# scorbiclife/LifeAPI

Measured on AMD Instinct MI355X. Metric: 64x64 universe-generations/sec (+ cell-updates/sec) at 1/2/4/8 MI355X, higher is better.
Workload: dtype u64

## Files before the change

### lifeapi_amd/csrc/device.hpp

```cpp
#pragma once

#include <hip/hip_runtime.h>

#include <cstdint>

#include "common.hpp"

namespace lifeapi_impl {


struct W {
  uint32_t lo, hi;
};

__device__ __forceinline__ W split(uint64_t v) { return W{(uint32_t)v, (uint32_t)(v >> 32)}; }
__device__ __forceinline__ uint64_t join(W w) { return (uint64_t)w.lo | ((uint64_t)w.hi << 32); }

__device__ __forceinline__ W rot_up(W a) {
  return W{__builtin_amdgcn_alignbit(a.lo, a.hi, 31), __builtin_amdgcn_alignbit(a.hi, a.lo, 31)};
}
__device__ __forceinline__ W rot_dn(W a) {
  return W{__builtin_amdgcn_alignbit(a.hi, a.lo, 1), __builtin_amdgcn_alignbit(a.lo, a.hi, 1)};
}

constexpr uint32_t TA = 0xF0, TB = 0xCC, TC = 0xAA;
constexpr uint32_t kXor3 = (TA ^ TB ^ TC) & 0xFF;
constexpr uint32_t kMaj = ((TA & TB) | (TA & TC) | (TB & TC)) & 0xFF;
constexpr uint32_t kCarry2 = (TA ^ (TB & TC)) & 0xFF;
constexpr uint32_t kLive = ((TA ^ TB) & (TC | TA)) & 0xFF;

template <uint32_t TT>
__device__ __forceinline__ uint32_t lut3(uint32_t a, uint32_t b, uint32_t c) {
  return __builtin_amdgcn_bitop3_b32(a, b, c, TT);
}
template <uint32_t TT>
__device__ __forceinline__ W lut3(W a, W b, W c) {
  return W{lut3<TT>(a.lo, b.lo, c.lo), lut3<TT>(a.hi, b.hi, c.hi)};
}


enum Xchg { XDPP = 0, XLDS = 1, XBPERM = 2, XMIX = 3, XMIX1 = 4, XMIX3 = 5, XLDSR = 6, XLDSR3 = 7, XASM = 8 };
constexpr bool uses_lds(int x) { return x == XLDS || x == XLDSR || x == XLDSR3 || x == XASM; }

__device__ __forceinline__ uint32_t dpp_prev(uint32_t v) {
  return (uint32_t)__builtin_amdgcn_mov_dpp((int)v, 0x13C, 0xF, 0xF, true);
}
__device__ __forceinline__ uint32_t dpp_next(uint32_t v) {
  return (uint32_t)__builtin_amdgcn_mov_dpp((int)v, 0x134, 0xF, 0xF, true);
}
__device__ __forceinline__ uint32_t bperm_prev(uint32_t v, int lane) {
  return (uint32_t)__builtin_amdgcn_ds_bpermute(((lane + kWave - 1) & (kWave - 1)) << 2, (int)v);
}
__device__ __forceinline__ uint32_t bperm_next(uint32_t v, int lane) {
  return (uint32_t)__builtin_amdgcn_ds_bpermute(((lane + 1) & (kWave - 1)) << 2, (int)v);
}

template <int X>
__device__ __forceinline__ void neighbour_cols(W a, W &L, W &R, uint64_t *slot, int lane);

template <int X>
__device__ __forceinline__ void neighbours(W c0, W c1, W &L0, W &R0, W &L1, W &R1,
                                           uint64_t *slot, int lane) {
  if constexpr (X != XLDS) {
    neighbour_cols<X>(c0, L0, R0, slot, lane);
    neighbour_cols<X>(c1, L1, R1, slot, lane);
  } else {
    uint64_t *s = slot;
    s[lane] = join(c0);
    s[kWave + lane] = join(c1);
    __builtin_amdgcn_wave_barrier();
    const int xp = (lane + kWave - 1) & (kWave - 1), xn = (lane + 1) & (kWave - 1);
    L0 = split(s[xp]);
    R0 = split(s[xn]);
    L1 = split(s[kWave + xp]);
    R1 = split(s[kWave + xn]);
    __builtin_amdgcn_wave_barrier();
  }
}

template <int X>
__device__ __forceinline__ void neighbour_cols(W a, W &L, W &R, uint64_t *slot, int lane) {
  if constexpr (X == XDPP) {
    L = W{dpp_prev(a.lo), dpp_prev(a.hi)};
    R = W{dpp_next(a.lo), dpp_next(a.hi)};
  } else if constexpr (X == XBPERM) {
    L = W{bperm_prev(a.lo, lane), bperm_prev(a.hi, lane)};
    R = W{bperm_next(a.lo, lane), bperm_next(a.hi, lane)};
  } else if constexpr (X == XMIX) {
    L = W{dpp_prev(a.lo), dpp_prev(a.hi)};
    R = W{bperm_next(a.lo, lane), bperm_next(a.hi, lane)};
  } else if constexpr (X == XMIX1) {
    L = W{dpp_prev(a.lo), dpp_prev(a.hi)};
    R = W{dpp_next(a.lo), bperm_next(a.hi, lane)};
  } else if constexpr (X == XMIX3) {
    L = W{dpp_prev(a.lo), bperm_prev(a.hi, lane)};
    R = W{bperm_next(a.lo, lane), bperm_next(a.hi, lane)};
  } else if constexpr (X == XLDSR || X == XLDSR3) {
    uint64_t *s = slot;
    s[lane] = join(a);
    __builtin_amdgcn_wave_barrier();
    R = split(s[(lane + 1) & (kWave - 1)]);
    if constexpr (X == XLDSR) {
      L = W{dpp_prev(a.lo), dpp_prev(a.hi)};
    } else {
      const uint32_t *s32 = reinterpret_cast<const uint32_t *>(s);
      L = W{dpp_prev(a.lo), s32[2 * ((lane + kWave - 1) & (kWave - 1)) + 1]};
    }
    __builtin_amdgcn_wave_barrier();
  } else {
    uint64_t *s = slot;
    s[lane] = join(a);
    __builtin_amdgcn_wave_barrier();
    L = split(s[(lane + kWave - 1) & (kWave - 1)]);
    R = split(s[(lane + 1) & (kWave - 1)]);
    __builtin_amdgcn_wave_barrier();
  }
}

constexpr uint32_t kLe1 = (~kMaj) & 0xFF;
constexpr uint32_t kNae = ((TA ^ TB) | (TB ^ TC)) & 0xFF;
constexpr uint32_t kEven = (~kXor3) & 0xFF;
constexpr uint32_t kT1 = 0x34, kT2 = 0x58, kT3 = 0x28;

constexpr uint32_t kN1 = 0xE9, kN4 = 0x52, kN6 = 0xE0;
__device__ __forceinline__ uint32_t life_tail6(uint32_t h0u, uint32_t h0, uint32_t h0d, uint32_t h1u,
                                               uint32_t h1, uint32_t h1d, uint32_t a) {
  const uint32_t g1 = lut3<kN1>(h1, h1u, h1d);
  const uint32_t g2 = lut3<kMaj>(h1d, h1u, h0d);
  const uint32_t g3 = lut3<kNae>(h0d, h0u, h0);
  const uint32_t g4 = lut3<kN4>(g3, g2, g1);
  const uint32_t g5 = lut3<kXor3>(h0, h0d, h0u);
  return lut3<kN6>(g4, g5, a);
}
__device__ __forceinline__ uint32_t life_tail7(uint32_t h0u, uint32_t h0, uint32_t h0d, uint32_t h1u,
                                               uint32_t h1, uint32_t h1d, uint32_t a) {
  const uint32_t s0 = lut3<kLe1>(h0u, h0, h0d), s1 = lut3<kNae>(h0u, h0, h0d);
  const uint32_t s2 = lut3<kLe1>(h1u, h1, h1d), s3 = lut3<kEven>(h1u, h1, h1d);
  const uint32_t t1 = lut3<kT1>(s0, s1, a);
  const uint32_t t2 = lut3<kT2>(s2, a, t1);
  return lut3<kT3>(s1, s3, t2);
}
template <int NET>
__device__ __forceinline__ uint32_t life_tail(uint32_t h0u, uint32_t h0, uint32_t h0d, uint32_t h1u,
                                              uint32_t h1, uint32_t h1d, uint32_t a) {
  static_assert(NET == 6 || NET == 7, "tails: 6 or 7 LUTs");
  if constexpr (NET == 6) return life_tail6(h0u, h0, h0d, h1u, h1, h1d, a);
  else return life_tail7(h0u, h0, h0d, h1u, h1, h1d, a);
}

typedef uint64_t u64x2 __attribute__((ext_vector_type(2)));

template <bool NT>
__device__ __forceinline__ W ld(const uint64_t *p) {
  if constexpr (NT) return split(__builtin_nontemporal_load(p));
  else return split(*p);
}
template <bool NT>
__device__ __forceinline__ void st(uint64_t *p, W v) {
  if constexpr (NT) __builtin_nontemporal_store(join(v), p);
  else *p = join(v);
}

__device__ __forceinline__ uint64_t mix64(uint64_t z) {
  z = (z ^ (z >> 30)) * 0xBF58476D1CE4E5B9ULL;
  z = (z ^ (z >> 27)) * 0x94D049BB133111EBULL;
  return z ^ (z >> 31);
}

template <int CTRL>
__device__ __forceinline__ uint32_t dpp_mov(uint32_t v) {
  return (uint32_t)__builtin_amdgcn_update_dpp(0, (int)v, CTRL, 0xF, 0xF, false);
}
template <int CTRL>
__device__ __forceinline__ uint64_t dpp_mov64(uint64_t v) {
  return (uint64_t)dpp_mov<CTRL>((uint32_t)v) | ((uint64_t)dpp_mov<CTRL>((uint32_t)(v >> 32)) << 32);
}
__device__ __forceinline__ uint32_t wave_sum_u32_dpp(uint32_t v) {
  v += dpp_mov<0xB1>(v);
  v += dpp_mov<0x4E>(v);
  v += dpp_mov<0x141>(v);
  v += dpp_mov<0x140>(v);
  return (uint32_t)__builtin_amdgcn_readlane(v, 0) + (uint32_t)__builtin_amdgcn_readlane(v, 16) +
         (uint32_t)__builtin_amdgcn_readlane(v, 32) + (uint32_t)__builtin_amdgcn_readlane(v, 48);
}
__device__ __forceinline__ uint32_t lane_id_fresh() {
  uint32_t l;
  asm volatile("v_mbcnt_lo_u32_b32 %0, -1, 0\n v_mbcnt_hi_u32_b32 %0, -1, %0" : "=v"(l));
  return l;
}

__device__ __forceinline__ uint32_t wave_or_u32_dpp(uint32_t v) {
  v |= dpp_mov<0xB1>(v);
  v |= dpp_mov<0x4E>(v);
  v |= dpp_mov<0x141>(v);
  v |= dpp_mov<0x140>(v);
  return (uint32_t)__builtin_amdgcn_readlane(v, 0) | (uint32_t)__builtin_amdgcn_readlane(v, 16) |
         (uint32_t)__builtin_amdgcn_readlane(v, 32) | (uint32_t)__builtin_amdgcn_readlane(v, 48);
}
__device__ __forceinline__ uint64_t wave_sum_u64_dpp(uint64_t v) {
  auto step = [&](auto mov) __attribute__((always_inline)) {
    v += (uint64_t)mov((uint32_t)v) | ((uint64_t)mov((uint32_t)(v >> 32)) << 32);
  };
  step(dpp_mov<0xB1>);
  step(dpp_mov<0x4E>);
  step(dpp_mov<0x141>);
  step(dpp_mov<0x140>);
  uint64_t t = 0;
#pragma unroll
  for (int r = 0; r < 4; ++r)
    t += (uint64_t)(uint32_t)__builtin_amdgcn_readlane((uint32_t)v, 16 * r) |
         ((uint64_t)(uint32_t)__builtin_amdgcn_readlane((uint32_t)(v >> 32), 16 * r) << 32);
  return t;
}

__device__ __forceinline__ uint32_t wave_sum_u32(uint32_t v) {
#pragma unroll
  for (int off = 32; off > 0; off >>= 1) v += __shfl_xor(v, off, kWave);
  return v;
}
__device__ __forceinline__ uint64_t wave_sum_u64(uint64_t v) {
#pragma unroll
  for (int off = 32; off > 0; off >>= 1) v += __shfl_xor(v, off, kWave);
  return v;
}

__device__ __forceinline__ uint32_t wave_excl_scan(uint32_t v, int lane) {
  uint32_t inc = v;
#pragma unroll
  for (int off = 1; off < kWave; off <<= 1) {
    const uint32_t t = __shfl_up(inc, off, kWave);
    if (lane >= off) inc += t;
  }
  return inc - v;
}
__device__ __forceinline__ uint64_t below_lane(int lane) { return (1ull << lane) - 1; }
__device__ __forceinline__ int last_set(uint64_t m) { return m ? 63 - __builtin_clzll(m) : -1; }


__device__ __forceinline__ uint64_t xcd_chunk_block() {
  const uint32_t b = blockIdx.x, nb = gridDim.x, q = nb >> 3, r = nb & 7u, x = b & 7u;
  return (uint64_t)x * q + (x < r ? x : r) + (b >> 3);
}
template <bool CHUNK>
__device__ __forceinline__ uint64_t block_index() {
  if constexpr (CHUNK) return xcd_chunk_block();
  else return blockIdx.x;
}

__device__ __forceinline__ uint64_t rotr64(uint64_t v, uint32_t k) {
  return (v >> k) | (v << ((64 - k) & 63));
}
__device__ __forceinline__ void care_window(uint64_t rm, uint32_t &y0, uint32_t &h) {
  y0 = 0;
  h = 1;
  if (rm == 0) return;
  uint64_t run[6];
  run[0] = ~rm;
#pragma unroll
  for (int k = 1; k < 6; ++k) run[k] = run[k - 1] & rotr64(run[k - 1], 1u << (k - 1));
  uint64_t cur = ~0ull;
  uint32_t len = 0;
#pragma unroll
  for (int k = 5; k >= 0; --k) {
    const uint64_t t = cur & rotr64(run[k], len);
    if (t) cur = t, len += 1u << k;
  }
  h = 64 - len;
  y0 = len ? ((uint32_t)__builtin_ctzll(cur) + len) & 63 : 0;
}
constexpr int kWaitVm0 = 0x0F70, kWaitVm1 = 0x0F71, kWaitVm5 = 0x0F75, kWaitVm6 = 0x0F76, kWaitVm9 = 0x0F79,
              kWaitVm11 = 0x0F7B, kWaitLgkm0 = 0xC07F;

__device__ __forceinline__ bool wave_contains(W s, W w, W u) {
  const uint32_t dlo = (s.lo ^ w.lo) & (w.lo | u.lo), dhi = (s.hi ^ w.hi) & (w.hi | u.hi);
  return __ballot((dlo | dhi) != 0u) == 0ull;
}


}
```

### lifeapi_amd/csrc/step.hip

```cpp
#include <algorithm>

#include "cone_launch.hpp"
#include "contains_kernels.hpp"
#include "launch.hpp"
#include "step_kernels.hpp"

using namespace lifeapi_impl;

namespace {

using StepFn = void (*)(const uint64_t *, uint64_t *, uint64_t, uint32_t, uint64_t);

constexpr uint64_t kCachedUniverses = 1ull << 22;
constexpr uint64_t kCap7Universes = 1ull << 20;
constexpr uint64_t kCap6Universes = 1ull << 21;
constexpr int kStreamResidentBlocks = 6;
int stream_resident_blocks(uint64_t n) {
  return n < kCap7Universes ? 0 : n < kCap6Universes ? 7 : kStreamResidentBlocks;
}
constexpr uint64_t kOrderMinUniverses = 3ull << 16;
constexpr uint64_t kPlainBytes = 256ull << 20;
constexpr uint64_t kFilterOrderUniverses = 1ull << 21;
constexpr const char *kStreamName =
    "k_step<dpp, 4 universes/wave, nt loads, 7-LUT network; alternating order, the last min(256 MiB, half) of "
    "each launch stored plain, the rest nt>";
constexpr const char *kStreamBigName =
    "k_step<dpp, 4 universes/wave, nt, 7-LUT network; each XCD a contiguous eighth, one order>";
struct StepLaunch {
  StepFn fn;
  uint64_t universes_per_wave;
  int resident_blocks;
  bool alternate;
  uint64_t plain_bytes;
  const char *name;
  uint32_t flags;
};
StepLaunch shipped_step(uint32_t gens, uint64_t n) {
  if (gens <= 2 && n > kCachedUniverses)
    return {k_step<XDPP, 4, true, 3, true, true>, 4, stream_resident_blocks(n), false, 0, kStreamBigName, kXcdChunk};
  if (gens <= 2)
    return {k_step<XDPP, 4, true, 3, true, true>, 4, stream_resident_blocks(n), true,
            std::min<uint64_t>(kPlainBytes, n * 512 / 2), kStreamName, 0u};
  if (gens < 32)
    return {k_step_split<8, 1, true, 6, kAsmLoop>, 4, 0, false, 0,
            "k_step_split<8-way split, 4 universes/wave, nt, 6-LUT tail, assembly loop>", 0u};
  return {k_step_split<8, 1, false, 6, kAsmLoop>, 4, 0, false, 0,
          "k_step_split<8-way split, 4 universes/wave, 6-LUT tail, assembly loop>", 0u};
}


constexpr int kFilterIterBlocksPerCU = 16;
constexpr int kSplitIterBlocksPerCU = 32;

using SplitFn = void (*)(const uint64_t *, uint64_t *, const uint64_t *, const uint64_t *, uint32_t *, uint64_t,
                         uint32_t, uint32_t);

int filter_cone(const uint64_t *d_in, const uint64_t *d_wanted, const uint64_t *d_unwanted, uint32_t *d_first_gen,
                size_t n, uint32_t generations, void *stream) {
  return launch_cone_adapt<kConeSets, true, uint32_t, true>(d_in, d_wanted, d_unwanted, d_first_gen, n, generations, 0,
                                                            (hipStream_t)stream, kConeAdaptBlocksPerCU, kWave,
                                                            kConeAdaptBlocksPerCU);
}

int filter_iterated(const uint64_t *d_in, const uint64_t *d_wanted, const uint64_t *d_unwanted,
                    uint32_t *d_first_gen, size_t n, uint32_t generations, void *stream) {
  const SplitFn fn = aligned16(d_in) ? k_step_contains_split<8, kContainsNet, kContainsAll, true, true>
                                     : k_step_contains_split<8, kContainsNet, kContainsAll, false, true>;
  return launch(fn, "k_step_contains_split launch", Grid{(n + 3) / 4, kFilterIterBlocksPerCU}, stream,
                kWritesNoBatch, d_in, nullptr, d_wanted, d_unwanted, d_first_gen, n, generations, kConeIterColumns);
}

int final_split_pair(const uint64_t *d_in, uint64_t *d_final, const uint64_t *d_wanted, const uint64_t *d_unwanted,
                     uint32_t *d_first_gen, size_t n, uint32_t generations, void *stream) {
  int cus = 0, rc = device_cus(cus);
  Written w{d_final, (uint64_t)n * 512};
  for (const SplitFn fn : {SplitFn(k_step_contains_split<8, kContainsNet, kContainsLo>),
                           SplitFn(k_step_contains_split<8, kContainsNet, kContainsHi>)}) {
    if (rc != LIFEAPI_OK) return rc;
    rc = launch(fn, "k_step_contains_split launch", Grid{(n + 3) / 4, kSplitIterBlocksPerCU, 0, cus}, stream, w, d_in,
                d_final, d_wanted, d_unwanted, d_first_gen, n, generations, 0u);
    w.recorded = true;
  }
  return rc;
}

int final_stream(const uint64_t *d_in, uint64_t *d_final, const uint64_t *d_wanted, const uint64_t *d_unwanted,
                 uint32_t *d_first_gen, size_t n, uint32_t generations, void *stream) {
  const uint64_t groups = (n + 7) / 8;
  const bool keyed = n <= kFilterOrderUniverses && n >= kOrderMinUniverses;
  const LaunchOrder o = launch_order(d_in, d_final, (uint64_t)n * 512, groups, 8 * 512, keyed,
                                     keyed ? std::min<uint64_t>(kPlainBytes, n * 512 / 2) : 0);
  return launch(k_step_contains<8>, "k_step_contains launch", Grid{groups}, stream, o.written, d_in, d_final,
                d_wanted, d_unwanted, d_first_gen, n, generations | (o.reverse ? kReverse : 0u), o.plain_from);
}

}

extern "C" {

const char *lifeapi_step_kernel_name_n(uint32_t generations, size_t n) {
  return shipped_step(generations, n).name;
}
const char *lifeapi_step_kernel_name(uint32_t generations) { return shipped_step(generations, 1).name; }

int lifeapi_step_batch_dev(const uint64_t *d_in, uint64_t *d_out, size_t n, uint32_t generations,
                           void *stream) {
  int rc = check_batch(d_in, d_out, n);
  if (rc != LIFEAPI_OK || n == 0) return rc;
  const StepLaunch l = shipped_step(generations, n);
  const uint64_t waves = (n + l.universes_per_wave - 1) / l.universes_per_wave;
  const LaunchOrder o = launch_order(d_in, d_out, (uint64_t)n * 512, waves, l.universes_per_wave * 512,
                                     l.alternate && n >= kOrderMinUniverses, l.plain_bytes);
  return launch(l.fn, "k_step launch", Grid{waves, 0, l.resident_blocks, 0, true}, stream, o.written, d_in, d_out, n,
                generations | (o.reverse ? kReverse : 0u) | l.flags, o.plain_from);
}

int lifeapi_step_contains_batch_dev(const uint64_t *d_in, uint64_t *d_final,
                                    const uint64_t *d_wanted, const uint64_t *d_unwanted,
                                    uint32_t *d_first_gen, size_t n, uint32_t generations,
                                    void *stream) {
  if (n == 0) return LIFEAPI_OK;
  if (!d_in || !d_wanted || !d_unwanted || !d_first_gen || !aligned8(d_in) ||
      !aligned8(d_wanted) || !aligned8(d_unwanted) || ((uintptr_t)d_first_gen & 3u))
    return fail(LIFEAPI_E_INVALID, "bad pointer to lifeapi_step_contains_batch_dev%s");
  if (!d_final) {
    if (generations <= 2) return filter_cone(d_in, d_wanted, d_unwanted, d_first_gen, n, generations, stream);
    return filter_iterated(d_in, d_wanted, d_unwanted, d_first_gen, n, generations, stream);
  }
  const int rc = check_batch(d_in, d_final, n);
  if (rc != LIFEAPI_OK) return rc;
  if (generations > 2)
    return final_split_pair(d_in, d_final, d_wanted, d_unwanted, d_first_gen, n, generations, stream);
  return final_stream(d_in, d_final, d_wanted, d_unwanted, d_first_gen, n, generations, stream);
}

}
```

### lifeapi_amd/csrc/step_kernels.hpp

```cpp
#pragma once

#include "life_gen.hpp"
#include "split_layout.hpp"
#include "split_asm.inc"

namespace lifeapi_impl {
namespace {

constexpr uint32_t kReverse = 1u << 31;
constexpr uint32_t kXcdChunk = 1u << 30;

template <int X, int U, bool NT, int RULE, bool NTS, bool FULL>
__device__ __forceinline__ void step_group(const uint64_t *in, uint64_t *out, uint64_t n, uint32_t gens,
                                           uint64_t u0, bool nts, uint64_t *slot, int lane) {
  W a[U];
#pragma unroll
  for (int k = 0; k < U; ++k)
    a[k] = (FULL || u0 + k < n) ? ld<NT>(in + (u0 + k) * kWave + lane) : W{0u, 0u};
  if constexpr (RULE == 4) {
#pragma unroll
    for (int k = 0; k < U; ++k) a[k] = to_eo(a[k]);
  }
  for (uint32_t g = 0; g < gens; ++g) {
#pragma unroll
    for (int k = 0; k < U; ++k) a[k] = life_gen<X, RULE>(a[k], slot + k * 2 * kWave, lane);
  }
  if constexpr (RULE == 4) {
#pragma unroll
    for (int k = 0; k < U; ++k) a[k] = from_eo(a[k]);
  }
  if (nts) {
#pragma unroll
    for (int k = 0; k < U; ++k)
      if (FULL || u0 + k < n) st<NTS>(out + (u0 + k) * kWave + lane, a[k]);
  } else {
    if constexpr (FULL) asm volatile("; plain-stored tail");
#pragma unroll
    for (int k = 0; k < U; ++k)
      if (FULL || u0 + k < n) st<false>(out + (u0 + k) * kWave + lane, a[k]);
    if constexpr (FULL) asm volatile("; plain-stored tail end");
  }
}

template <int X, int U, bool NT, int RULE, bool NTS, bool ONESHOT = false>
__device__ __forceinline__ void step_body(const uint64_t *in, uint64_t *out, uint64_t n, uint32_t gens,
                                          uint64_t plain_from) {
  __shared__ uint64_t lds[uses_lds(X) ? kWavesPerBlock * U * 2 * kWave : 1];
  const int lane = threadIdx.x & (kWave - 1);
  const int wib = __builtin_amdgcn_readfirstlane(threadIdx.x / kWave);
  const bool rev = (gens & kReverse) != 0;
  const uint64_t blk = (gens & kXcdChunk) ? xcd_chunk_block() : (uint64_t)blockIdx.x;
  gens &= ~(kReverse | kXcdChunk);
  const uint64_t groups = (n + U - 1) / U, wstride = (uint64_t)gridDim.x * kWavesPerBlock;
  uint64_t *slot = lds + (uses_lds(X) ? wib * U * 2 * kWave : 0);
  auto group = [&](uint64_t grp) __attribute__((always_inline)) {
    const uint64_t u0 = (rev ? groups - 1 - grp : grp) * U;
    if (u0 + U <= n) step_group<X, U, NT, RULE, NTS, true>(in, out, n, gens, u0, grp < plain_from, slot, lane);
    else step_group<X, U, NT, RULE, NTS, false>(in, out, n, gens, u0, grp < plain_from, slot, lane);
  };
  const uint64_t first = blk * kWavesPerBlock + wib;
  if constexpr (ONESHOT) {
    if (first < groups) group(first);
  } else {
    for (uint64_t grp = first; grp < groups; grp += wstride) group(grp);
  }
}

template <int X, int U, bool NT, int RULE, bool NTS = NT, bool ONESHOT = false>
__global__ __launch_bounds__(kBlock) void k_step(const uint64_t *in, uint64_t *out, uint64_t n,
                                                 uint32_t gens, uint64_t plain_from) {
  step_body<X, U, NT, RULE, NTS, ONESHOT>(in, out, n, gens, plain_from);
}
template <int X, int U, bool NT, int RULE, bool NTS = NT, bool ONESHOT = false>
__global__ __launch_bounds__(kBlock) void k_step_ab(const uint64_t *in, uint64_t *out, uint64_t n,
                                                    uint32_t gens, uint64_t plain_from) {
  step_body<X, U, NT, RULE, NTS, ONESHOT>(in, out, n, gens, plain_from);
}

template <int U, int RULE, bool NTS, bool WIDE>
__device__ __forceinline__ void step_body_dma(const uint64_t *in, uint64_t *out, uint64_t n, uint32_t gens,
                                              uint64_t plain_from) {
  static_assert(U % 2 == 0, "pairs of universes per 16-byte load");
  __shared__ uint64_t img_all[kWavesPerBlock][U * kWave];
  const int lane = threadIdx.x & (kWave - 1);
  const int wib = __builtin_amdgcn_readfirstlane(threadIdx.x / kWave);
  uint64_t *img = img_all[wib];
  const bool rev = (gens & kReverse) != 0;
  const uint64_t blk = (gens & kXcdChunk) ? xcd_chunk_block() : (uint64_t)blockIdx.x;
  gens &= ~(kReverse | kXcdChunk);
  const uint64_t groups = (n + U - 1) / U, wstride = (uint64_t)gridDim.x * kWavesPerBlock;
  for (uint64_t grp = blk * kWavesPerBlock + wib; grp < groups; grp += wstride) {
    const uint64_t u0 = (rev ? groups - 1 - grp : grp) * U;
#pragma unroll
    for (int i = 0; i < U / 2; ++i) {
      uint64_t u = u0 + 2 * i + (lane >> 5);
      if (u >= n) u = n - 1;
      const char *src = reinterpret_cast<const char *>(in + u * kWave) + (lane & 31) * 16;
      __builtin_amdgcn_global_load_lds((const __attribute__((address_space(1))) void *)src,
                                       (__attribute__((address_space(3))) void *)(img + i * 2 * kWave), 16, 0, 2);
    }
    __builtin_amdgcn_s_waitcnt(kWaitVm0);
    W a[U];
#pragma unroll
    for (int k = 0; k < U; ++k) a[k] = split(img[k * kWave + lane]);
    for (uint32_t g = 0; g < gens; ++g) {
#pragma unroll
      for (int k = 0; k < U; ++k) a[k] = life_gen<XDPP, RULE>(a[k], nullptr, lane);
    }
    const bool nt = NTS && grp < plain_from;
    if constexpr (WIDE) {
#pragma unroll
      for (int k = 0; k < U; ++k) img[k * kWave + lane] = join(a[k]);
      const u64x2 *src = reinterpret_cast<const u64x2 *>(img) + lane;
#pragma unroll
      for (int i = 0; i < U / 2; ++i) {
        const uint64_t u = u0 + 2 * i + (lane >> 5);
        const u64x2 v = src[i * kWave];
        u64x2 *dst = reinterpret_cast<u64x2 *>(out + u * kWave) + (lane & 31);
        if (u < n) {
          if (nt) __builtin_nontemporal_store(v, dst);
          else *dst = v;
        }
      }
    } else {
#pragma unroll
      for (int k = 0; k < U; ++k)
        if (u0 + k < n) {
          if (nt) st<true>(out + (u0 + k) * kWave + lane, a[k]);
          else st<false>(out + (u0 + k) * kWave + lane, a[k]);
        }
    }
  }
}

template <int U, int RULE, bool NTS, bool WIDE>
__global__ __launch_bounds__(kBlock) void k_step_dma(const uint64_t *in, uint64_t *out, uint64_t n, uint32_t gens,
                                                     uint64_t plain_from) {
  step_body_dma<U, RULE, NTS, WIDE>(in, out, n, gens, plain_from);
}

constexpr int kPipe = -1;
constexpr int kAsmLoop = -3;
template <int S, int G, bool NT, int NET, int D = 0, int V = 0, int WPB = kWavesPerBlock>
__global__ __launch_bounds__(WPB * kWave) void k_step_split(const uint64_t *in, uint64_t *out, uint64_t n,
                                                            uint32_t gens, uint64_t ) {
  constexpr int P = S / 2;
  __shared__ uint32_t lds[WPB * G * S * kWave];
  const int lane = threadIdx.x & (kWave - 1);
  const int wib = __builtin_amdgcn_readfirstlane(threadIdx.x / kWave);
  const uint64_t per_wave = (uint64_t)G * P;
  const uint64_t stride = (uint64_t)gridDim.x * WPB * per_wave;
  for (uint64_t u0 = ((uint64_t)blockIdx.x * WPB + wib) * per_wave; u0 < n; u0 += stride) {
    uint32_t r[G][S];
#pragma unroll
    for (int g = 0; g < G; ++g) {
      W c[P];
#pragma unroll
      for (int u = 0; u < P; ++u) {
        const uint64_t x = u0 + g * P + u;
        c[u] = x < n ? ld<NT>(in + x * kWave + lane) : W{0u, 0u};
      }
      Split<S>::load(c, r[g]);
    }
    if constexpr (D == kPipe) {
#pragma unroll
      for (int g = 0; g < G; ++g) gens_split_pipe<S, NET>(r[g], lds + (wib * G + g) * S * kWave, lane, gens);
    } else if constexpr (D == kAsmLoop) {
      static_assert(S == 8 && NET == 6 && G <= 2, "split_asm.inc is rule 11, one or two groups");
      const uint32_t base = (uint32_t)(uintptr_t)(const __attribute__((address_space(3))) void *)(
          lds + wib * G * S * kWave);
      const uint32_t self = base + lane * 16u, prev = base + ((lane + kWave - 1) & (kWave - 1)) * 16u,
                     next = base + ((lane + 1) & (kWave - 1)) * 16u;
      if constexpr (G == 2) split_gens_asm2(r[0], r[1], gens, self, prev, next);
      else if constexpr (V == 1) split_gens_asm_v1(r[0], gens, self, prev, next);
      else if constexpr (V == 2) split_gens_asm_v2(r[0], gens, self, prev, next);
      else if constexpr (V == 3) split_gens_asm_v3(r[0], gens, self, prev, next);
      else split_gens_asm_v0(r[0], gens, self, prev, next);
    } else {
      for (uint32_t it = 0; it < gens; ++it) {
#pragma unroll
        for (int g = 0; g < G; ++g) gen_split<S, NET, D>(r[g], lds + (wib * G + g) * S * kWave, lane);
      }
    }
#pragma unroll
    for (int g = 0; g < G; ++g) {
      W c[P];
      Split<S>::store(r[g], c);
#pragma unroll
      for (int u = 0; u < P; ++u) {
        const uint64_t x = u0 + g * P + u;
        if (x < n) st<NT>(out + x * kWave + lane, c[u]);
      }
    }
  }
}

}
}
```

Baseline: 7.220 billion.

## Unify XCD-chunked step scheduling with alternating order and plain-store tail

Moves the block-to-group mapping into a shared host/device helper, step_take, that combines XCD-contiguous chunk placement, reversed order and the plain-vs-nontemporal store split. The XCD chunking now also applies to medium sizes (512K to 2M universes) and to large sizes, which now also alternate direction between launches and keep a plain-stored tail. The aim is to keep each XCD's L2 and the MALL holding data that the next launch reads first. The lower 7-block residency cap threshold is also moved. The plain decision is keyed on the unchunked block index, so the plainly stored groups may not line up with the ones read first next launch.

```diff
diff --git a/lifeapi_amd/csrc/device.hpp b/lifeapi_amd/csrc/device.hpp
--- a/lifeapi_amd/csrc/device.hpp
+++ b/lifeapi_amd/csrc/device.hpp
@@ -5,6 +5,7 @@
 #include <cstdint>
 
 #include "common.hpp"
+#include "step_order.hpp"
 
 namespace lifeapi_impl {
 
@@ -237,10 +238,7 @@
 __device__ __forceinline__ int last_set(uint64_t m) { return m ? 63 - __builtin_clzll(m) : -1; }
 
 
-__device__ __forceinline__ uint64_t xcd_chunk_block() {
-  const uint32_t b = blockIdx.x, nb = gridDim.x, q = nb >> 3, r = nb & 7u, x = b & 7u;
-  return (uint64_t)x * q + (x < r ? x : r) + (b >> 3);
-}
+__device__ __forceinline__ uint64_t xcd_chunk_block() { return xcd_chunk_place(blockIdx.x, gridDim.x); }
 template <bool CHUNK>
 __device__ __forceinline__ uint64_t block_index() {
   if constexpr (CHUNK) return xcd_chunk_block();
diff --git a/lifeapi_amd/csrc/step.hip b/lifeapi_amd/csrc/step.hip
--- a/lifeapi_amd/csrc/step.hip
+++ b/lifeapi_amd/csrc/step.hip
@@ -11,8 +11,13 @@
 
 using StepFn = void (*)(const uint64_t *, uint64_t *, uint64_t, uint32_t, uint64_t);
 
-constexpr uint64_t kCachedUniverses = 1ull << 22;
-constexpr uint64_t kCap7Universes = 1ull << 20;
+constexpr uint64_t kChunkMinUniverses = 1ull << 19;
+constexpr uint64_t kChunkStopUniverses = 1ull << 21;
+constexpr uint64_t kChunkBigUniverses = 1ull << 22;
+bool stream_chunks(uint64_t n) {
+  return (n >= kChunkMinUniverses && n < kChunkStopUniverses) || n >= kChunkBigUniverses;
+}
+constexpr uint64_t kCap7Universes = 1ull << 19;
 constexpr uint64_t kCap6Universes = 1ull << 21;
 constexpr int kStreamResidentBlocks = 6;
 int stream_resident_blocks(uint64_t n) {
@@ -23,9 +28,10 @@
 constexpr uint64_t kFilterOrderUniverses = 1ull << 21;
 constexpr const char *kStreamName =
     "k_step<dpp, 4 universes/wave, nt loads, 7-LUT network; alternating order, the last min(256 MiB, half) of "
-    "each launch stored plain, the rest nt>";
+    "each launch stored plain, the rest nt; each XCD a contiguous eighth from 512K up to 2M and from 4M universes>";
 constexpr const char *kStreamBigName =
-    "k_step<dpp, 4 universes/wave, nt, 7-LUT network; each XCD a contiguous eighth, one order>";
+    "k_step<dpp, 4 universes/wave, nt loads, 7-LUT network; each XCD a contiguous eighth, the order reversed from "
+    "launch to launch, the last 32 MiB of every eighth stored plain, the rest nt>";
 struct StepLaunch {
   StepFn fn;
   uint64_t universes_per_wave;
@@ -36,11 +42,10 @@
   uint32_t flags;
 };
 StepLaunch shipped_step(uint32_t gens, uint64_t n) {
-  if (gens <= 2 && n > kCachedUniverses)
-    return {k_step<XDPP, 4, true, 3, true, true>, 4, stream_resident_blocks(n), false, 0, kStreamBigName, kXcdChunk};
   if (gens <= 2)
     return {k_step<XDPP, 4, true, 3, true, true>, 4, stream_resident_blocks(n), true,
-            std::min<uint64_t>(kPlainBytes, n * 512 / 2), kStreamName, 0u};
+            std::min<uint64_t>(kPlainBytes, n * 512 / 2), n > kChunkBigUniverses ? kStreamBigName : kStreamName,
+            stream_chunks(n) ? kXcdChunk : 0u};
   if (gens < 32)
     return {k_step_split<8, 1, true, 6, kAsmLoop>, 4, 0, false, 0,
             "k_step_split<8-way split, 4 universes/wave, nt, 6-LUT tail, assembly loop>", 0u};
diff --git a/lifeapi_amd/csrc/step_kernels.hpp b/lifeapi_amd/csrc/step_kernels.hpp
--- a/lifeapi_amd/csrc/step_kernels.hpp
+++ b/lifeapi_amd/csrc/step_kernels.hpp
@@ -3,6 +3,7 @@
 #include "life_gen.hpp"
 #include "split_layout.hpp"
 #include "split_asm.inc"
+#include "step_order.hpp"
 
 namespace lifeapi_impl {
 namespace {
@@ -48,21 +49,23 @@
   __shared__ uint64_t lds[uses_lds(X) ? kWavesPerBlock * U * 2 * kWave : 1];
   const int lane = threadIdx.x & (kWave - 1);
   const int wib = __builtin_amdgcn_readfirstlane(threadIdx.x / kWave);
-  const bool rev = (gens & kReverse) != 0;
-  const uint64_t blk = (gens & kXcdChunk) ? xcd_chunk_block() : (uint64_t)blockIdx.x;
+  const bool rev = (gens & kReverse) != 0, chunk = (gens & kXcdChunk) != 0;
   gens &= ~(kReverse | kXcdChunk);
-  const uint64_t groups = (n + U - 1) / U, wstride = (uint64_t)gridDim.x * kWavesPerBlock;
+  const uint64_t groups = (n + U - 1) / U;
   uint64_t *slot = lds + (uses_lds(X) ? wib * U * 2 * kWave : 0);
-  auto group = [&](uint64_t grp) __attribute__((always_inline)) {
-    const uint64_t u0 = (rev ? groups - 1 - grp : grp) * U;
-    if (u0 + U <= n) step_group<X, U, NT, RULE, NTS, true>(in, out, n, gens, u0, grp < plain_from, slot, lane);
-    else step_group<X, U, NT, RULE, NTS, false>(in, out, n, gens, u0, grp < plain_from, slot, lane);
+  auto take = [&](uint64_t pass) __attribute__((always_inline)) {
+    const StepTake t = step_take(blockIdx.x, gridDim.x, wib, pass, groups, chunk, rev, plain_from);
+    if (t.index >= groups) return false;
+    const uint64_t u0 = t.group * U;
+    if (u0 + U <= n) step_group<X, U, NT, RULE, NTS, true>(in, out, n, gens, u0, !t.plain, slot, lane);
+    else step_group<X, U, NT, RULE, NTS, false>(in, out, n, gens, u0, !t.plain, slot, lane);
+    return true;
   };
-  const uint64_t first = blk * kWavesPerBlock + wib;
   if constexpr (ONESHOT) {
-    if (first < groups) group(first);
+    take(0);
   } else {
-    for (uint64_t grp = first; grp < groups; grp += wstride) group(grp);
+    for (uint64_t pass = 0; take(pass); ++pass) {
+    }
   }
 }
 
diff --git a/lifeapi_amd/csrc/step_order.hpp b/lifeapi_amd/csrc/step_order.hpp
--- /dev/null
+++ b/lifeapi_amd/csrc/step_order.hpp
@@ -0,0 +1,29 @@
+#pragma once
+
+#include "common.hpp"
+
+#if defined(__HIPCC__)
+#define LIFEAPI_HD __host__ __device__ __forceinline__
+#else
+#define LIFEAPI_HD inline
+#endif
+
+namespace lifeapi_impl {
+
+LIFEAPI_HD uint64_t xcd_chunk_place(uint32_t b, uint32_t nb) {
+  const uint32_t q = nb >> 3, r = nb & 7u, x = b & 7u;
+  return (uint64_t)x * q + (x < r ? x : r) + (b >> 3);
+}
+
+struct StepTake {
+  uint64_t index, group;
+  bool plain;
+};
+LIFEAPI_HD StepTake step_take(uint32_t b, uint32_t nb, uint32_t wib, uint64_t pass, uint64_t groups, bool chunk,
+                              bool reverse, uint64_t plain_from) {
+  const uint64_t off = wib + pass * nb * kWavesPerBlock;
+  const uint64_t index = (chunk ? xcd_chunk_place(b, nb) : (uint64_t)b) * kWavesPerBlock + off;
+  return {index, reverse ? groups - 1 - index : index, (uint64_t)b * kWavesPerBlock + off >= plain_from};
+}
+
+}
```

New measurement: 7.320 billion (median of 6 runs). +1.4%, better.
